# nmdp-bioinformatics/py-graph-imputation

Hardware: NVIDIA B200
Metric: subjects_per_sec (higher is better)
Workload: dtype f64

## Files before the change

py-graph-imputation_b200/csrc/grimb200.cu:

```cuda
#include <cuda_runtime.h>
#include <cub/cub.cuh>

#include <chrono>
#include <cstdio>
#include <cstring>
#include <mutex>
#include <string>
#include <vector>

#include "grimb_plan.h"

using namespace grimb;

static thread_local std::string g_err;
static int fail(int code, const std::string& msg) {
  g_err = msg;
  return code;
}
#define CK(call)                                                                          \
  do {                                                                                    \
    cudaError_t e_ = (call);                                                              \
    if (e_ != cudaSuccess)                                                                \
      return fail(GRIMB_E_CUDA, std::string(#call) + ": " + cudaGetErrorString(e_));      \
  } while (0)
// ... 1655 lines not shown
    }
    const bool drain_now = qn >= PQ_DRAIN;
    if (drain_now) drain_issue(q, X, qh, qn, lane, d);
    uint32_t p1[2];
#pragma unroll
    for (int u = 0; u < 2; ++u) {
      p1[u] = GRIMB_NONE;
      bool more = pr[u] && fidx_step(w[u], key[u], sec[u], true, p1[u]);
      while (more) {
        sec[u] = (sec[u] + 1) & X.sec_mask;
        fidx_sector(X.keys + 4ull * sec[u], w[u]);
        more = fidx_step(w[u], key[u], sec[u], false, p1[u]);
      }
    }
    const bool last = stride >= S - s0;
#pragma unroll
    for (int u = 0; u < 2; ++u) {
      nf[u] = 0x8000u;
      if (!last && S - s0 - stride > (uint32_t)(2 * u + half)) {
        nk[u] = __ldg(reinterpret_cast<const uint4*>(B.packed_keys) + s0 + stride + 2 * u + half);
        nf[u] = B.packed_flags[s0 + stride + 2 * u + half];
      }
    }
    if (drain_now) {
      const uint32_t n = drain_finish(q, d, X, qh, mid, worklist, worklist_n, extra, extra_n, extra_cap, lane);
      qh += n;
      qn -= n;
      __syncwarp();
    }
    uint32_t base = qh + qn;
#pragma unroll
    for (int u = 0; u < 2; ++u) {
      const uint32_t s = s0 + 2 * u + half;
      const uint32_t fl = cf[u];
      const bool inb = S - s0 > (uint32_t)(2 * u + half);
      const bool shape = inb && !(fl & 0x8000u) && nchain_ok;
      const bool same = (fl & 31u) == 0u;
      const bool hit = p1[u] != GRIMB_NONE;
      const uint32_t enq = __ballot_sync(FULL, hit && !same);
      const uint32_t hh = (enq >> (half << 4)) & 0xFFFFu;
      if (hit && !same) {
        const uint32_t e = (base + __popc(enq & lt)) & (PQ_CAP - 1u);
        q.key[e] = key2[u];
        q.p1[e] = p1[u];
        q.s[e] = s;
        q.ph[e] = (uint8_t)i;
      }
      base += __popc(enq);
      if (i == 0 && inb) {
        if (!shape) {
          if (fl & 0x8000u)
            O.r.compact[s] = make_compact(GRIMB_ST_SKIPPED, GRIMB_KIND_GENERAL, 0, 0xFFFFFFFFu, 0.0);
          else
            worklist[atomicAdd(worklist_n, 1u)] = s;
          mid.head[s] = FastHead{0u, 0u, make_uint2(0u, 0u)};
        } else if (same) {
          mid.head[s] = FastHead{1u | (hit ? (1u << 2) | (1u << 16) : 0u) | (1u << 7), 0u, make_uint2(p1[u], p1[u])};
        } else if (hh == 0u) {
          mid.head[s] = FastHead{1u, 0u, make_uint2(0u, 0u)};
        }
      }
    }
    qn = base - qh;
    __syncwarp();
    while (qn >= PQ_HIGH) {
      drain_issue(q, X, qh, qn, lane, d);
      const uint32_t n = drain_finish(q, d, X, qh, mid, worklist, worklist_n, extra, extra_n, extra_cap, lane);
      qh += n;
      qn -= n;
      __syncwarp();
    }
    if (last) break;
    s0 += stride;
  }
  while (qn > 0) {
    drain_issue(q, X, qh, qn, lane, d);
    const uint32_t n = drain_finish(q, d, X, qh, mid, worklist, worklist_n, extra, extra_n, extra_cap, lane);
    qh += n;
    qn -= n;
    __syncwarp();
  }
}

struct LongCand {
  FastPair pr;
  double p;
  bool valid;
};

__device__ __forceinline__ void long_cand(LongCand& c, const FastExtra* ex, const double* __restrict__ fslot, uint32_t q,
                                          uint32_t ncand, double m, bool same) {
  c.valid = q < ncand;
  double2 v = make_double2(0.0, 0.0);
  if (c.valid) {
    const uint2 pp = ex->p[q];
    v.x = __ldg(fslot + pp.x);
    v.y = __ldg(fslot + pp.y);
  }
  c.pr.f = v.x;
  c.pr.f2 = v.y;
  c.pr.same = same;
  c.pr.mpos = c.valid && m > 0;
  c.pr.y = m * c.pr.f2;
  const double t = fmin(c.pr.f2, same ? c.pr.y * 0.5 : c.pr.y);
  const double b = c.pr.f * t;
  const bool tiny = !(b > 1.0e-280);
  c.pr.lo = tiny ? -1.0 : b * (1.0 - 0x1p-50);
  c.pr.hi = tiny ? __longlong_as_double(0x7ff0000000000000LL) : b * (1.0 + 0x1p-50);
  c.p = v.x * v.y * m;
  if (!same) c.p = c.p * 2;
}

__device__ __forceinline__ double shfl_double(double v, int src) {
  const long long b = __double_as_longlong(v);
  const int lo = __shfl_sync(0xFFFFFFFFu, (int)(b & 0xFFFFFFFFll), src), hi = __shfl_sync(0xFFFFFFFFu, (int)(b >> 32), src);
  return __longlong_as_double(((long long)hi << 32) | (unsigned int)lo);
}

struct ScoreLong {
  double total, e_fin;
  uint32_t n_acc, evals;
};

__device__ __noinline__ void score_long_eval(const FastExtra* ex, const double* fslot, uint32_t ncand, double m, bool same,
                                             const double* chain, int nchain, ScoreLong& o) {
  const int lane = threadIdx.x & 31;
  LongCand c;
  long_cand(c, ex, fslot, (uint32_t)lane, ncand, m, same);
  uint32_t rq = 99;
  if (c.pr.mpos) {
    int r = 0;
    while (r < nchain && chain[r] >= c.pr.hi) ++r;
    while (r < nchain && !c.pr.accept(chain[r])) ++r;
    if (r < nchain) rq = (uint32_t)r;
  }
  const uint32_t rs = __reduce_min_sync(0xFFFFFFFFu, rq);
  o.total = 0.0;
  o.e_fin = 0.0;
  o.n_acc = 0;
  if (rs == 99) {
    o.evals = ncand * (uint32_t)nchain;
    return;
  }
  o.evals = ncand * (rs + 1);
  bool acc = rq <= rs;
  if (chain[rs] > 0) {
    double mx = acc ? c.p : 0.0;
#pragma unroll
    for (int d = 16; d > 0; d >>= 1) {
      const double y = shfl_double(mx, lane ^ d);
      mx = y > mx ? y : mx;
    }
    o.e_fin = mx / 100000;
    acc = c.pr.accept(o.e_fin);
    o.evals += ncand;
  }
  uint32_t am = __ballot_sync(0xFFFFFFFFu, acc);
  o.n_acc = (uint32_t)__popc(am);
  bool first = true;
  while (am) {
    const int j = __ffs(am) - 1;
    am &= am - 1;
    const double pj = shfl_double(c.p, j);
    o.total = first ? pj : o.total + pj;
    first = false;
  }
}

__device__ __noinline__ void score_long_rows(const FastExtra* ex, const double* fslot, uint32_t ncand, double m, bool same,
                                             double e_fin, uint32_t cmask, uint32_t np, uint64_t* words) {
  const int lane = threadIdx.x & 31;
  LongCand c;
  long_cand(c, ex, fslot, (uint32_t)lane, ncand, m, same);
  const bool acc = c.pr.accept(e_fin);
  uint32_t am = __ballot_sync(0xFFFFFFFFu, acc);
  uint32_t rank = 0;
  while (am) {
    const int j = __ffs(am) - 1;
    am &= am - 1;
    const double pj = shfl_double(c.p, j);
    if (pj > c.p || (pj == c.p && j < lane)) ++rank;
  }
  uint32_t lo = 0, hi = 0;
  if (acc && rank < np) {
    const uint32_t id = __fns(cmask, 0, lane + 1) & 15u;
    if (rank < 8) lo = id << (4 * rank);
    else hi = id << (4 * (rank - 8));
    words[2 + rank] = (uint64_t)__double_as_longlong(c.p);
  }
  lo = __reduce_or_sync(0xFFFFFFFFu, lo);
  hi = __reduce_or_sync(0xFFFFFFFFu, hi);
  if (lane == 0) {
    words[0] = (uint64_t)np;
    words[1] = (uint64_t)lo | ((uint64_t)hi << 32);
  }
}

#ifndef FASTSCORE_MIN_BLOCKS
#define FASTSCORE_MIN_BLOCKS 8
#endif
__global__ void __launch_bounds__(128, FASTSCORE_MIN_BLOCKS)
k_fast_score(TablesView T, const FastIndex X, const GrimbConfig* __restrict__ cfg, GrimbBatch B, OutArrays O,
             const FastMid mid, const FastExtra* __restrict__ extra, uint32_t* worklist, unsigned int* worklist_n,
             uint32_t s_begin) {
  __shared__ double s_chain[FAST_MAX_ROUNDS];
  __shared__ int s_nchain;
  const int lane = threadIdx.x & 31;
  GrimbResults& R = O.r;
  const bool want_u = cfg->output_umug != 0, want_p = cfg->output_pmug != 0, planb = cfg->planb != 0;
  const uint32_t lim_r = (uint32_t)cfg->n_results;
  if (threadIdx.x == 0) {
    double e = cfg->epsilon;
    int n = 0;
    while (e > 0 && n < FAST_MAX_ROUNDS) {
      e /= 10;
      if (e < 1.0e-9) e = 0.0;
      s_chain[n++] = e;
    }
    s_nchain = (e > 0) ? -1 : n;
  }
  __syncthreads();
  const int nchain = s_nchain;
  const uint64_t S = (uint64_t)B.n_subjects;
  const uint64_t nthreads = (uint64_t)gridDim.x * blockDim.x;
  unsigned long long evals_sum = 0;
  for (uint64_t s0 = (uint64_t)s_begin + ((uint64_t)blockIdx.x * blockDim.x + threadIdx.x) - lane; s0 < S; s0 += nthreads) {
    const uint64_t s = s0 + lane;
    bool ready = false;
    double m = 0.0;
    uint32_t fl = 0, xslot = 0;
    uint32_t cmask = 0;
    uint2 p0 = make_uint2(0u, 0u);
    if (s < S) {
      const uint4 h1 = *reinterpret_cast<const uint4*>(mid.head + s);
      const uint32_t pi = batch_prior(B, s);
      m = __ldg(B.priors + pi);
      fl = h1.x;
      xslot = h1.y;
      p0 = make_uint2(h1.z, h1.w);
      cmask = fl >> 16;
      ready = (fl & 3u) == 1u;
    }
    const uint32_t ncand_all = ready ? ((fl >> 2) & 31u) : 0u;
    const bool long_form = ncand_all > (uint32_t)FAST_CMAX;
    const uint32_t ncand = long_form ? 0u : ncand_all;
    const bool same = (fl >> 7) & 1u;
    const bool mpos = m > 0;
    ScoreLong sl;
    sl.total = sl.e_fin = 0.0;
    sl.n_acc = sl.evals = 0;
    for (uint32_t lm = __ballot_sync(0xFFFFFFFFu, long_form); lm; lm &= lm - 1) {
      const int o = __ffs(lm) - 1;
      ScoreLong r;
      score_long_eval(extra + __shfl_sync(0xFFFFFFFFu, xslot, o), X.fslot, __shfl_sync(0xFFFFFFFFu, ncand_all, o), shfl_double(m, o),
                      __shfl_sync(0xFFFFFFFFu, (int)same, o) != 0, s_chain, nchain, r);
      if (lane == o) sl = r;
    }
    double pf[FAST_CMAX], pf2[FAST_CMAX], prob[FAST_CMAX];
    uint32_t rq[FAST_CMAX];
    bool acc[FAST_CMAX];
    uint32_t r_star = 99;
    uint2 pp[FAST_CMAX];
    pp[0] = p0;
#pragma unroll
    for (int q = 1; q < FAST_CMAX; ++q) pp[q] = (uint32_t)q < ncand ? mid.more[s].p[q - 1] : make_uint2(0u, 0u);
#pragma unroll
    for (int q = 0; q < FAST_CMAX; ++q) {
      pf[q] = pf2[q] = 0.0;
      if ((uint32_t)q < ncand) {
        pf[q] = __ldg(X.fslot + pp[q].x);
        pf2[q] = __ldg(X.fslot + pp[q].y);
      }
    }
#pragma unroll
    for (int q = 0; q < FAST_CMAX; ++q) {
      prob[q] = 0.0;
      rq[q] = 99;
      acc[q] = false;
      if ((uint32_t)q < ncand) {
        const double2 v = make_double2(pf[q], pf2[q]);
        FastPair pr;
        pr.f = v.x;
        pr.f2 = v.y;
        pr.same = same;
        pr.mpos = mpos;
        pr.y = m * pr.f2;
        const double t = fmin(pr.f2, same ? pr.y * 0.5 : pr.y);
        const double b = pr.f * t;
        const bool tiny = !(b > 1.0e-280);
        pr.lo = tiny ? -1.0 : b * (1.0 - 0x1p-50);
        pr.hi = tiny ? __longlong_as_double(0x7ff0000000000000LL) : b * (1.0 + 0x1p-50);
        double p = v.x * v.y * m;
        if (!same) p = p * 2;
        prob[q] = p;
        if (mpos) {
          int r = 0;
          while (r < nchain && s_chain[r] >= pr.hi) ++r;
          while (r < nchain && !pr.accept(s_chain[r])) ++r;
          if (r < nchain) rq[q] = (uint32_t)r;
        }
        r_star = rq[q] < r_star ? rq[q] : r_star;
      }
    }
    uint32_t evals = 0, n_acc = 0;
    if (r_star == 99) {
      evals = ncand * (uint32_t)nchain;
    } else {
      evals = ncand * (r_star + 1);
      if (s_chain[r_star] > 0) {
        double mx = 0.0;
#pragma unroll
        for (int q = 0; q < FAST_CMAX; ++q)
          if (rq[q] <= r_star && prob[q] > mx) mx = prob[q];
        const double eps = mx / 100000;
#pragma unroll
        for (int q = 0; q < FAST_CMAX; ++q)
          if ((uint32_t)q < ncand) {
            FastPair pr;
            pr.f = pf[q];
            pr.f2 = pf2[q];
            pr.same = same;
            pr.mpos = mpos;
            pr.y = m * pr.f2;
            const double t = fmin(pr.f2, same ? pr.y * 0.5 : pr.y);
            const double b = pr.f * t;
            const bool tiny = !(b > 1.0e-280);
            pr.lo = tiny ? -1.0 : b * (1.0 - 0x1p-50);
            pr.hi = tiny ? __longlong_as_double(0x7ff0000000000000LL) : b * (1.0 + 0x1p-50);
            acc[q] = pr.accept(eps);
          }
        evals += ncand;
      } else {
#pragma unroll
        for (int q = 0; q < FAST_CMAX; ++q) acc[q] = rq[q] <= r_star;
      }
    }
    double total = 0.0;
    bool first = true;
#pragma unroll
    for (int q = 0; q < FAST_CMAX; ++q)
      if (acc[q]) {
        total = first ? prob[q] : total + prob[q];
        first = false;
        ++n_acc;
      }
    if (long_form) {
      total = sl.total;
      n_acc = sl.n_acc;
      evals = sl.evals;
    }
    if (want_u && want_p) evals *= 2;
    bool done = ready;
    if (ready && n_acc == 0 && planb) {
      worklist[atomicAdd(worklist_n, 1u)] = (uint32_t)s;
      done = false;
    }
    if (done) evals_sum += evals;
    const uint32_t np = (done && n_acc != 0 && want_p) ? (n_acc < lim_r ? n_acc : lim_r) : 0u;
    const uint32_t nw = long_form ? (np ? np + 2u : 0u) : ((np != 0u && n_acc >= 2u) ? np : 0u);
    uint32_t sc = nw;
#pragma unroll
    for (int d = 1; d < 32; d <<= 1) {
      const uint32_t a = __shfl_up_sync(0xFFFFFFFFu, sc, d);
      if (lane >= d) sc += a;
    }
    const uint32_t wtot = __shfl_sync(0xFFFFFFFFu, sc, 31);
    unsigned long long wb = 0;
    if (wtot) {
      if (lane == 31) wb = atomicAdd(O.word_counter, (unsigned long long)wtot);
      wb = __shfl_sync(0xFFFFFFFFu, wb, 31);
    }
    const uint64_t my = wb + (sc - nw);
    const bool fits = (int64_t)(wb + wtot) <= R.word_capacity;
    for (uint32_t lm = __ballot_sync(0xFFFFFFFFu, long_form && done && np && fits); lm; lm &= lm - 1) {
      const int o = __ffs(lm) - 1;
      const uint32_t ph = __shfl_sync(0xFFFFFFFFu, cmask, o);
      const uint64_t at = (uint64_t)__shfl_sync(0xFFFFFFFFu, (uint32_t)my, o) |
                          ((uint64_t)__shfl_sync(0xFFFFFFFFu, (uint32_t)(my >> 32), o) << 32);
      score_long_rows(extra + __shfl_sync(0xFFFFFFFFu, xslot, o), X.fslot, __shfl_sync(0xFFFFFFFFu, ncand_all, o), shfl_double(m, o),
                      __shfl_sync(0xFFFFFFFFu, (int)same, o) != 0, shfl_double(sl.e_fin, o), ph, __shfl_sync(0xFFFFFFFFu, np, o),
                      R.words + at);
    }
    if (!done) continue;
    uint32_t phases = 0;
    uint32_t mm = cmask;
#pragma unroll
    for (int q = 0; q < FAST_CMAX; ++q) {
      const uint32_t pid = (uint32_t)(__ffs(mm) - 1) & 15u;
      mm &= mm - 1;
      if (acc[q]) {
        uint32_t rank = 0;
#pragma unroll
        for (int j = 0; j < FAST_CMAX; ++j)
          if (acc[j] && (prob[j] > prob[q] || (prob[j] == prob[q] && j < q))) ++rank;
        if (rank < np) {
          phases |= pid << (4 * rank);
          if (nw && fits) R.words[my + rank] = (uint64_t)__double_as_longlong(prob[q]);
        }
      }
    }
    const GrimbCompact c = make_compact(GRIMB_ST_OK, GRIMB_KIND_SIMPLE | (n_acc ? GRIMB_KIND_HAS_RESULTS : 0u) |
                                        (nw ? GRIMB_KIND_WORDS : 0u) | ((long_form ? (np ? 15u : 0u) : np) << 4), phases,
                                        (uint32_t)my, total);
    *reinterpret_cast<uint4*>(R.compact + s) = *reinterpret_cast<const uint4*>(&c);
  }
#pragma unroll
  for (int d = 16; d > 0; d >>= 1) evals_sum += __shfl_xor_sync(0xFFFFFFFFu, evals_sum, d);
  if (lane == 0 && evals_sum) atomicAdd(O.evals_counter, evals_sum);
}

#endif

constexpr int TY_WARPS = 8;
constexpr int TY_VP = 4;
#ifndef TY_MIN_BLOCKS
#define TY_MIN_BLOCKS 4
#endif
constexpr int TY_MAX_ROUNDS = 40;

struct __align__(16) TyLists {
  uint16_t ph[TY_VP];
  uint16_t ph_pad[4];
  double f1s[TY_VP][32];
  double f2s[TY_VP][32];
  double pm2[TY_VP][32];
  double xs[32];
  uint8_t p1s[TY_VP][32];
  uint8_t p2s[TY_VP][32];
  uint8_t n1[TY_VP], n2[TY_VP];
};

static inline size_t ty_bytes_per_warp(int P) {
  const size_t G = (size_t)P * (P + 1) / 2;
  return (sizeof(TyLists) + G * 12 + 15) & ~(size_t)15;
}

__global__ void __launch_bounds__(TY_WARPS * 32, TY_MIN_BLOCKS)
k_impute_typed(TablesView T, const GrimbConfig* __restrict__ cfg, GrimbBatch B, OutArrays O, uint32_t* worklist,
               unsigned int* worklist_n, uint32_t per_warp, uint32_t s_begin) {
  extern __shared__ __align__(16) unsigned char ty_smem[];
  __shared__ double s_chain[TY_MAX_ROUNDS];
  __shared__ int s_nchain;
  const uint32_t FULLM = 0xFFFFFFFFu;
  const int lane = threadIdx.x & 31, warp = threadIdx.x >> 5;
  const int L = T.L, P = T.P;
  const int G = P * (P + 1) / 2;
  TyLists& W = *reinterpret_cast<TyLists*>(ty_smem + (size_t)warp * per_warp);
  double* gsum = reinterpret_cast<double*>(ty_smem + (size_t)warp * per_warp + sizeof(TyLists));
  uint16_t* gslot = reinterpret_cast<uint16_t*>(gsum + G);
  uint16_t* gpair = gslot + G;
  GrimbResults& R = O.r;
  const bool want_u = cfg->output_umug != 0, want_p = cfg->output_pmug != 0;
  const uint32_t lim_r = (uint32_t)cfg->n_results, lim_p = (uint32_t)cfg->n_pop_results;
  const int K = cfg->max_haps_in_phase;
  if (threadIdx.x == 0) {
    double e = cfg->epsilon;
    int n = 0;
    while (e > 0 && n < TY_MAX_ROUNDS) {
      e /= 10;
      if (e < 1.0e-9) e = 0.0;
      s_chain[n++] = e;
    }
    s_nchain = (e > 0) ? -1 : n;
  }
  __syncthreads();
  const int nchain = s_nchain;
  const uint32_t full = (1u << L) - 1u;
  const uint32_t nphase = 1u << (L - 1);
  const uint64_t S = (uint64_t)B.n_subjects;
  unsigned long long evals_sum = 0;
  unsigned long long n_probes = 0, n_hits = 0, n_vecs = 0;
  for (uint64_t s = (uint64_t)s_begin + (uint64_t)blockIdx.x * TY_WARPS + warp; s < S; s += (uint64_t)gridDim.x * TY_WARPS) {
    const uint32_t typed = batch_typed(B, s, full);
    if (typed == 0) {
      if (lane == 0) R.compact[s] = make_compact(GRIMB_ST_SKIPPED, GRIMB_KIND_GENERAL, 0, 0xFFFFFFFFu, 0.0);
      continue;
    }
    const bool is_packed = B.packed_keys != nullptr;
    const uint32_t al_off = is_packed ? 0u : B.allele_off[s];
    const bool shape = typed == full && nchain >= 0 && (is_packed || B.allele_off[s + 1] - al_off == 2u * (uint32_t)L);
    uint32_t pairs[GRIMB_MAX_LOCI];
    uint32_t het = 0;
    if (shape) {
// ... 326 lines not shown
  out_idx[i] = s;
}

__global__ void k_snapshot(const unsigned long long* __restrict__ cnt, unsigned long long* out, int n) {
  if ((int)threadIdx.x < n) out[threadIdx.x] = cnt[threadIdx.x];
  __threadfence_system();
}

enum {
  CNT_WORK = 0,
  CNT_WORKLIST = 1,
  CNT_BUCKETS = 2,
  CNT_OVERFLOW = 4,
  CNT_SLOT_TICKET = 5,
  CNT_WORK2 = 6,
  CNT_CHUNK_END = 8,
  CNT_HAP = 8,
  CNT_POP = 9,
  CNT_WORDS = 10,
  CNT_GENERAL = 11,
  CNT_EVALS = 12,
  CNT_PROBES = 13,
  CNT_N = 16
};

struct GrimbEngine {
  const GrimbTables* tables;
  int device;
  int threads;
  int threads_fixed = 0;
  int64_t wide_cta_below = 2048;
  int split_heavy = 0;
  int n_ctas;
  uint64_t arena_per_cta;
  char* arena = nullptr;
  double* ones = nullptr;
  GrimbConfig* d_cfg = nullptr;
  unsigned long long* d_counters = nullptr;
  cudaStream_t stream = nullptr;
  cudaStream_t s_in = nullptr, s_out = nullptr;
  cudaEvent_t ev_in[GRIMB_MAX_CHUNKS], ev_k[GRIMB_MAX_CHUNKS];
  unsigned long long* h_cnt = nullptr;
  unsigned long long* h_cnt_dev = nullptr;
  int64_t host_chunk = 262144;
  GrimbConfig cfg_host;
  GrimbConfig cfg_dev;
  int cfg_sent = 0;
  unsigned long long* h_tail = nullptr;
  cudaStream_t pending_stream = nullptr;
  int pending = 0;
  cudaEvent_t ev_done = nullptr;
  int tail_queued = 0;
  int tail_expected = 0;
  GrimbBatch pend_batch;
  GrimbResults pend_res;
  int64_t launches = 0;
  DevBuf in[6], outb[5], in_mask;
  DevBuf worklist;
  DevBuf buckets;
  DevBuf gather;
  void* h_gather = nullptr;
  size_t h_gather_cap = 0;
  DevBuf pre_top, pre_meta;
  uint32_t pre_max = 0;
  int pre_K = 0;
  int sm_count = 0;
  int fast_path = 1;
  int fast_split = 1;
  int fast_probe = 2;
  int last_probe = -1;
  int timing = 1;
  int timing_host = 0;
  DevBuf mid;
  DevBuf overflow;
  cudaEvent_t ev_score[2] = {nullptr, nullptr};
  int ev_score_valid = 0;
  cudaEvent_t ev_slots[2] = {nullptr, nullptr};
  int ev_slots_valid = 0;
  cudaEvent_t ev[6] = {nullptr, nullptr, nullptr, nullptr, nullptr, nullptr};
  int ev_valid[3] = {0, 0, 0};
  double last_worklist = -1;
  int typed_ctas = 0;
  uint32_t typed_per_warp = 0;
  DevBuf geno_keys, geno_flags, geno_mask, geno_off, geno_alleles, geno_small, scan_tmp;
  unsigned long long* h_small = nullptr;
  cudaEvent_t ev_geno[4] = {nullptr, nullptr, nullptr, nullptr};
  int ev_geno_valid = 0;
  cudaEvent_t ev_rows[4] = {nullptr, nullptr, nullptr, nullptr};
  int ev_rows_valid = 0;
  DevBuf gl_in_off, gl_stage, gl_mask, gl_counts, gl_off, gl_alleles;
  cudaEvent_t ev_gl[4] = {nullptr, nullptr, nullptr, nullptr};
  int ev_gl_valid = 0;
};

extern "C" int grimb_engine_free(GrimbEngine* e);

static void set_l2_fetch_granularity() {
  const char* v = getenv("GRIMB_L2_FETCH");
  if (!v) return;
  const long x = atol(v);
  if (x != 32 && x != 64 && x != 128) return;
  if (cudaDeviceSetLimit(cudaLimitMaxL2FetchGranularity, (size_t)x) != cudaSuccess) cudaGetLastError();
}

extern "C" int grimb_engine_create(const GrimbTables* t, int64_t workspace_bytes_per_cta, GrimbEngine** out) {
  if (!t || !out || workspace_bytes_per_cta < (1 << 16)) return fail(GRIMB_E_ARG, "bad engine arguments");
  CK(cudaSetDevice(t->device));
  set_l2_fetch_granularity();
  GrimbEngine* e = new GrimbEngine();
  for (int i = 0; i < GRIMB_MAX_CHUNKS; ++i) e->ev_in[i] = e->ev_k[i] = nullptr;
  e->tables = t;
  e->device = t->device;
  e->threads = 128;
#define CKE(call)                                                                          \
  do {                                                                                     \
    cudaError_t e_ = (call);                                                               \
    if (e_ != cudaSuccess) {                                                               \
      grimb_engine_free(e);                                                                \
      return fail(GRIMB_E_CUDA, std::string(#call) + ": " + cudaGetErrorString(e_));       \
    }                                                                                      \
  } while (0)
  cudaDeviceProp prop;
  CKE(cudaGetDeviceProperties(&prop, t->device));
  int per_sm = 0;
  CKE(cudaOccupancyMaxActiveBlocksPerMultiprocessor(&per_sm, k_impute, e->threads, 0));
  if (per_sm < 1) per_sm = 1;
  size_t free_b = 0, total_b = 0;
  CKE(cudaMemGetInfo(&free_b, &total_b));
  int64_t n = (int64_t)prop.multiProcessorCount * per_sm;
  e->arena_per_cta = ((uint64_t)workspace_bytes_per_cta + 255ull) & ~255ull;
  while (n > prop.multiProcessorCount && (uint64_t)n * e->arena_per_cta > free_b / 2) n -= prop.multiProcessorCount;
  while (n > 1 && (uint64_t)n * e->arena_per_cta > free_b / 2) n /= 2;
  e->n_ctas = (int)n;
  cudaError_t ce = cudaMalloc((void**)&e->arena, (uint64_t)e->n_ctas * e->arena_per_cta);
  if (ce != cudaSuccess) {
    grimb_engine_free(e);
    return fail(GRIMB_E_NOMEM, std::string("engine arena: ") + cudaGetErrorString(ce));
  }
  const int P = t->h.P;
  std::vector<double> one((size_t)P * P, 1.0);
  CKE(cudaMalloc((void**)&e->ones, one.size() * 8));
  CKE(cudaMemcpy(e->ones, one.data(), one.size() * 8, cudaMemcpyHostToDevice));
  CKE(cudaMalloc((void**)&e->d_cfg, sizeof(GrimbConfig)));
  CKE(cudaMalloc((void**)&e->d_counters, CNT_N * sizeof(unsigned long long)));
  CKE(cudaStreamCreateWithFlags(&e->stream, cudaStreamNonBlocking));
  CKE(cudaStreamCreateWithFlags(&e->s_in, cudaStreamNonBlocking));
  CKE(cudaStreamCreateWithFlags(&e->s_out, cudaStreamNonBlocking));
  for (int i = 0; i < GRIMB_MAX_CHUNKS; ++i) {
    CKE(cudaEventCreateWithFlags(&e->ev_in[i], cudaEventDisableTiming));
    CKE(cudaEventCreateWithFlags(&e->ev_k[i], cudaEventDisableTiming));
  }
  CKE(cudaHostAlloc((void**)&e->h_cnt, (GRIMB_MAX_CHUNKS + 1) * CNT_N * sizeof(unsigned long long), cudaHostAllocMapped));
  CKE(cudaHostGetDevicePointer((void**)&e->h_cnt_dev, e->h_cnt, 0));
  CKE(cudaMallocHost((void**)&e->h_tail, CNT_N * sizeof(unsigned long long)));
  if (const char* hc = getenv("GRIMB_HOST_CHUNK")) {
    const long long v = atoll(hc);
    if (v >= 1024) e->host_chunk = v;
  }
  for (int i = 0; i < 6; ++i) CKE(cudaEventCreate(&e->ev[i]));
  e->sm_count = prop.multiProcessorCount;
  if (P <= 32) {
    e->typed_per_warp = (uint32_t)ty_bytes_per_warp(P);
    const size_t dyn = (size_t)e->typed_per_warp * TY_WARPS;
    CKE(cudaFuncSetAttribute(k_impute_typed, cudaFuncAttributeMaxDynamicSharedMemorySize,
                             (int)(ty_bytes_per_warp(32) * TY_WARPS)));
    int tb = 0;
    CKE(cudaOccupancyMaxActiveBlocksPerMultiprocessor(&tb, k_impute_typed, TY_WARPS * 32, dyn));
    e->typed_ctas = (tb < 1 ? 1 : tb) * prop.multiProcessorCount;
  }
  const char* fp = getenv("GRIMB_FAST");
  if (fp && fp[0] == '0') e->fast_path = 0;
  const char* fsp = getenv("GRIMB_FAST_SPLIT");
  if (fsp && fsp[0] == '0') e->fast_split = 0;
  const char* fpr = getenv("GRIMB_FAST_PROBE");
  if (fpr && fpr[0] == '1') e->fast_probe = 1;
  const char* kev = getenv("GRIMB_KERNEL_EVENTS");
  if (kev && kev[0] == '0') e->timing = 0;
  const char* hev = getenv("GRIMB_HOST_EVENTS");
  if (hev && hev[0] == '1') e->timing_host = 1;
  for (int i = 0; i < 2; ++i) CKE(cudaEventCreate(&e->ev_score[i]));
  for (int i = 0; i < 2; ++i) CKE(cudaEventCreate(&e->ev_slots[i]));
  CKE(cudaEventCreateWithFlags(&e->ev_done, cudaEventDisableTiming));
  for (int i = 0; i < 4; ++i) CKE(cudaEventCreate(&e->ev_geno[i]));
  for (int i = 0; i < 4; ++i) CKE(cudaEventCreate(&e->ev_rows[i]));
  for (int i = 0; i < 4; ++i) CKE(cudaEventCreate(&e->ev_gl[i]));
  CKE(cudaMallocHost((void**)&e->h_small, 8 * sizeof(unsigned long long)));
  e->pre_max = 4096;
  if (const char* gs = getenv("GRIMB_GROUP_SUBJECTS")) {
    const long long v = atoll(gs);
    if (v >= 0 && v <= (1 << 20)) e->pre_max = (uint32_t)v;
  }
  const char* th = getenv("GRIMB_THREADS");
  if (th) {
    int v = atoi(th);
    if (v >= 32 && v <= MAXT && v % 32 == 0) {
      e->threads = v;
      e->threads_fixed = 1;
    }
  }
  if (const char* wc = getenv("GRIMB_WIDE_CTA_BELOW")) e->wide_cta_below = atoll(wc);
  if (const char* sh = getenv("GRIMB_SPLIT_HEAVY")) {
    const int v = atoi(sh);
    if (v >= 0 && v < GRIMB_BUCKETS) e->split_heavy = v;
  }
#undef CKE
  *out = e;
  return GRIMB_OK;
}

extern "C" int grimb_engine_free(GrimbEngine* e) {
  if (!e) return GRIMB_OK;
  cudaSetDevice(e->device);
  if (e->stream) cudaStreamSynchronize(e->stream);
  cudaFree(e->arena);
  cudaFree(e->ones);
  cudaFree(e->d_cfg);
  cudaFree(e->d_counters);
  if (e->stream) cudaStreamDestroy(e->stream);
  if (e->s_in) cudaStreamDestroy(e->s_in);
  if (e->s_out) cudaStreamDestroy(e->s_out);
  for (int i = 0; i < GRIMB_MAX_CHUNKS; ++i) {
    if (e->ev_in[i]) cudaEventDestroy(e->ev_in[i]);
    if (e->ev_k[i]) cudaEventDestroy(e->ev_k[i]);
  }
  for (int i = 0; i < 6; ++i)
    if (e->ev[i]) cudaEventDestroy(e->ev[i]);
  for (int i = 0; i < 2; ++i)
    if (e->ev_score[i]) cudaEventDestroy(e->ev_score[i]);
  for (int i = 0; i < 2; ++i)
    if (e->ev_slots[i]) cudaEventDestroy(e->ev_slots[i]);
  if (e->ev_done) cudaEventDestroy(e->ev_done);
  for (int i = 0; i < 4; ++i) {
    if (e->ev_geno[i]) cudaEventDestroy(e->ev_geno[i]);
    if (e->ev_rows[i]) cudaEventDestroy(e->ev_rows[i]);
    if (e->ev_gl[i]) cudaEventDestroy(e->ev_gl[i]);
  }
  if (e->h_small) cudaFreeHost(e->h_small);
  if (e->h_gather) cudaFreeHost(e->h_gather);
  if (e->h_cnt) cudaFreeHost(e->h_cnt);
  if (e->h_tail) cudaFreeHost(e->h_tail);
  cudaGetLastError();
  delete e;
  return GRIMB_OK;
}

extern "C" int64_t grimb_engine_launches(const GrimbEngine* e) { return e ? e->launches : 0; }

extern "C" double grimb_engine_kernel_ms(const GrimbEngine* e, int which) {
  if (e && which == 3) return e->last_worklist;
  if (e && which == 6) return (double)e->last_probe;
  if (e && which >= 7 && which <= 9) {
    const cudaEvent_t* ev = which == 7 ? e->ev_geno : which == 8 ? e->ev_rows : e->ev_gl;
// ... 54 lines not shown
  CK(cudaStreamSynchronize(e->stream));
  e->cfg_host = *cfg;
  e->cfg_dev = *cfg;
  if (cfg->plan_a_only) e->cfg_dev.planb = 0;
  CK(cudaMemcpyAsync(e->d_cfg, &e->cfg_dev, sizeof(GrimbConfig), cudaMemcpyHostToDevice, st));
  CK(cudaStreamSynchronize(st));
  e->cfg_sent = 1;
  return GRIMB_OK;
}

static OutArrays out_arrays(GrimbEngine* e, const GrimbResults& r) {
  OutArrays O;
  O.r = r;
  O.hap_counter = e->d_counters + CNT_HAP;
  O.pop_counter = e->d_counters + CNT_POP;
  O.word_counter = e->d_counters + CNT_WORDS;
  O.general_counter = e->d_counters + CNT_GENERAL;
  O.evals_counter = e->d_counters + CNT_EVALS;
  O.probe_counters = e->d_counters + CNT_PROBES;
  return O;
}

static bool warp_kernels_apply(const GrimbEngine* e, const GrimbConfig* cfg, const GrimbBatch* batch) {
  if (!(e->fast_path && (!batch->phase_mask || batch->packed_keys) && !cfg->hap_pop_pair && !cfg->encounter_order)) return false;
  const TablesView& tv = e->tables->view;
#if GRIMB_KW == 1
  if (tv.L <= 5 && tv.P == 1) return true;
#endif
  return e->typed_ctas > 0;
}

static int launch_warp(GrimbEngine* e, const GrimbConfig* cfg, const GrimbBatch* batch, const OutArrays& O, cudaStream_t st,
                       bool tm, int64_t s_begin, int64_t s_end) {
  const int64_t n = s_end - s_begin;
  if (n <= 0 || !warp_kernels_apply(e, cfg, batch)) return GRIMB_OK;
  const TablesView& tv = e->tables->view;
  GrimbBatch rb = *batch;
  rb.n_subjects = s_end;
  CK(e->worklist.reserve((size_t)batch->n_subjects * 4 + 16));
  unsigned int* cnt = (unsigned int*)(e->d_counters + CNT_WORKLIST);
#if GRIMB_KW == 1
  if (tv.L <= 5 && tv.P == 1) {
    const uint64_t groups = ((uint64_t)n + FAST_WARPS * 2 - 1) / (FAST_WARPS * 2);
    if (e->fast_split) {
      const FastIndex& fidx = e->tables->fidx;
      if (!fidx.keys) return fail(GRIMB_E_ARG, "table has no fast-path index");
      CK(e->mid.reserve((size_t)batch->n_subjects * (sizeof(FastHead) + sizeof(FastMore)) + 256));
      FastMid midv;
      midv.head = (FastHead*)e->mid.p;
      midv.more = (FastMore*)((char*)e->mid.p + (((size_t)batch->n_subjects * sizeof(FastHead) + 127) & ~(size_t)127));
      double eps = cfg->epsilon;
      int nr = 0;
      while (eps > 0 && nr < FAST_MAX_ROUNDS) {
        eps /= 10;
        if (eps < 1.0e-9) eps = 0.0;
        ++nr;
      }
      uint64_t fgp = (uint64_t)e->sm_count * FASTPROBE_MIN_BLOCKS;
      if (fgp > groups) fgp = groups;
      const uint32_t extra_cap = (uint32_t)(batch->n_subjects / 16 + 1024);
      CK(e->overflow.reserve((size_t)extra_cap * sizeof(FastExtra) + 64));
      unsigned int* ovf_n = (unsigned int*)(e->d_counters + CNT_OVERFLOW);
      if (tm) CK(cudaEventRecord(e->ev[0], st));
      if (batch->packed_keys && e->fast_probe == 2) {
        uint64_t g2 = (uint64_t)e->sm_count * FASTPROBE2_MIN_BLOCKS;
        const uint64_t quads = ((uint64_t)n + FAST_WARPS * 4 - 1) / (FAST_WARPS * 4);
        if (g2 > quads) g2 = quads;
        k_fast_probe2<<<(unsigned)g2, FAST_WARPS * 32, 0, st>>>(tv, fidx, rb, O, midv, (uint32_t*)e->worklist.p, cnt,
                                                             (FastExtra*)e->overflow.p, ovf_n, extra_cap, eps > 0 ? 0 : 1,
                                                             (uint32_t)s_begin);
        e->last_probe = 2;
      } else if (batch->packed_keys) {
        k_fast_probe<true><<<(unsigned)fgp, FAST_WARPS * 32, 0, st>>>(tv, fidx, rb, O, midv, (uint32_t*)e->worklist.p, cnt,
                                                                    (FastExtra*)e->overflow.p, ovf_n, extra_cap, eps > 0 ? 0 : 1, (uint32_t)s_begin);
        e->last_probe = 1;
      } else {
        k_fast_probe<false><<<(unsigned)fgp, FAST_WARPS * 32, 0, st>>>(tv, fidx, rb, O, midv, (uint32_t*)e->worklist.p, cnt,
                                                                     (FastExtra*)e->overflow.p, ovf_n, extra_cap, eps > 0 ? 0 : 1, (uint32_t)s_begin);
        e->last_probe = 0;
      }
      CK(cudaGetLastError());
      if (tm) CK(cudaEventRecord(e->ev[1], st));
      uint64_t sg = ((uint64_t)n + 127) / 128;
      if (sg > (uint64_t)e->sm_count * 16) sg = (uint64_t)e->sm_count * 16;
      if (tm) CK(cudaEventRecord(e->ev_score[0], st));
      k_fast_score<<<(unsigned)sg, 128, 0, st>>>(tv, fidx, e->d_cfg, rb, O, midv, (const FastExtra*)e->overflow.p,
                                                (uint32_t*)e->worklist.p, cnt, (uint32_t)s_begin);
      CK(cudaGetLastError());
      if (tm) CK(cudaEventRecord(e->ev_score[1], st));
      e->ev_score_valid = tm;
      e->ev_valid[0] = tm;
      e->launches += 2;
    } else {
      uint64_t fg = (uint64_t)e->sm_count * FAST_MIN_BLOCKS;
      if (fg > groups) fg = groups;
      if (tm) CK(cudaEventRecord(e->ev[0], st));
      k_impute_fast<false><<<(unsigned)fg, FAST_WARPS * 32, 0, st>>>(tv, e->d_cfg, rb, O, (uint32_t*)e->worklist.p, cnt, nullptr,
                                                                    nullptr, (uint32_t)s_begin);
      CK(cudaGetLastError());
      if (tm) CK(cudaEventRecord(e->ev[1], st));
      e->ev_valid[0] = tm;
      e->launches += 1;
    }
    return GRIMB_OK;
  }
#endif
  uint64_t tg = ((uint64_t)n + TY_WARPS - 1) / TY_WARPS;
  if (tg > (uint64_t)e->typed_ctas) tg = (uint64_t)e->typed_ctas;
  if (tm) CK(cudaEventRecord(e->ev[4], st));
  k_impute_typed<<<(unsigned)tg, TY_WARPS * 32, (size_t)e->typed_per_warp * TY_WARPS, st>>>(
      tv, e->d_cfg, rb, O, (uint32_t*)e->worklist.p, cnt, e->typed_per_warp, (uint32_t)s_begin);
  CK(cudaGetLastError());
  if (tm) CK(cudaEventRecord(e->ev[5], st));
  e->ev_valid[2] = tm;
  e->launches += 1;
  return GRIMB_OK;
}

static int launch_tail(GrimbEngine* e, const GrimbConfig* cfg, const GrimbBatch* batch, const OutArrays& O, cudaStream_t st,
                       bool tm, int64_t n_tail = -1) {
  if (batch->n_subjects <= 0) return GRIMB_OK;
  const TablesView& tv = e->tables->view;
  const bool warp = warp_kernels_apply(e, cfg, batch);
  const uint32_t* wl = warp ? (const uint32_t*)e->worklist.p : nullptr;
  unsigned int* cnt = (unsigned int*)(e->d_counters + CNT_WORKLIST);
  const unsigned int* wl_n = warp ? cnt : nullptr;
  const uint64_t stride = (uint64_t)batch->n_subjects;
  CK(e->buckets.reserve((size_t)stride * 4 * GRIMB_BUCKETS + 16));
  unsigned int* bucket_n = (unsigned int*)(e->d_counters + CNT_BUCKETS);
  {
    uint64_t cg = (stride + 255) / 256;
    if (cg > (uint64_t)e->sm_count * 4) cg = (uint64_t)e->sm_count * 4;
    if (wl) cg = cg < 64 ? cg : 64;
    k_classify<<<(unsigned)cg, 256, 0, st>>>(*batch, tv.L, wl, wl_n, (uint32_t*)e->buckets.p, bucket_n, stride);
    CK(cudaGetLastError());
    e->launches += 1;
  }
  int grid = e->n_ctas;
  if ((int64_t)grid > batch->n_subjects) grid = (int)batch->n_subjects;
  int threads = e->threads;
  if (!e->threads_fixed && n_tail >= 0 && n_tail <= e->wide_cta_below && e->n_ctas >= 4) {
    threads = n_tail <= e->wide_cta_below / 8 ? 512 : 256;
    const int div = threads / 128;
    if (grid > e->n_ctas / div) grid = e->n_ctas / div;
  }
  PreView pv;
  memset(&pv, 0, sizeof(pv));
  if (e->pre_max > 0 && (!batch->phase_mask || batch->packed_keys)) {
    const uint32_t spp = 1u << tv.L;
    const uint32_t K = (uint32_t)cfg->max_haps_in_phase;
    uint64_t fit = e->pre_max;
    const uint64_t budget = 1ull << 31;
    const uint64_t per_subject = (uint64_t)spp * K * sizeof(TopItem);
    if (fit * per_subject > budget) fit = budget / per_subject;
    if ((int64_t)fit > batch->n_subjects) fit = (uint64_t)batch->n_subjects;
    if (fit > 0) {
      CK(e->pre_top.reserve(fit * per_subject + 16));
      CK(e->pre_meta.reserve(fit * spp * 12 + 16));
      pv.top = (TopItem*)e->pre_top.p;
      pv.n = (uint32_t*)e->pre_meta.p;
      pv.ne = pv.n + fit * spp;
      pv.ready = pv.ne + fit * spp;
      pv.max_subjects = (uint32_t)fit;
      pv.slots_per_subject = spp;
      pv.K = K;
      if (tm) CK(cudaEventRecord(e->ev_slots[0], st));
      k_impute<<<grid, threads, 0, st>>>(tv, e->d_cfg, *batch, O, e->arena, e->arena_per_cta, e->ones,
// ... 931 lines not shown
```

Measured before the change: 4.843 billion.

## Score multi-candidate subjects warp-cooperatively and size score grid by occupancy

Each thread now scores single-candidate subjects inline. Every subject with two or more candidates, short or long form, goes through a warp-cooperative loop in which each lane handles one candidate. This replaces the per-thread unrolled FAST_CMAX arrays and the rank loops, which should cut register pressure and divergence. The change also switches subject indices to 32-bit, skips the word-offset scan when no lane needs words, lowers the launch-bounds min blocks from 8 to 6, and sets the score grid from measured occupancy. The trade-off is more warp-serialised work when many subjects in a warp have multiple candidates.

```diff
diff --git a/py-graph-imputation_b200/csrc/grimb200.cu b/py-graph-imputation_b200/csrc/grimb200.cu
--- a/py-graph-imputation_b200/csrc/grimb200.cu
+++ b/py-graph-imputation_b200/csrc/grimb200.cu
@@ -1761,33 +1761,51 @@
   }
 }
 
-struct LongCand {
+__device__ __forceinline__ FastPair fast_pair(double f, double f2, double m, bool same) {
+  FastPair pr;
+  pr.f = f;
+  pr.f2 = f2;
+  pr.same = same;
+  pr.mpos = m > 0;
+  pr.y = m * f2;
+  const double t = fmin(f2, same ? pr.y * 0.5 : pr.y);
+  const double b = f * t;
+  const bool tiny = !(b > 1.0e-280);
+  pr.lo = tiny ? -1.0 : b * (1.0 - 0x1p-50);
+  pr.hi = tiny ? __longlong_as_double(0x7ff0000000000000LL) : b * (1.0 + 0x1p-50);
+  return pr;
+}
+
+__device__ __forceinline__ double fast_prob(double f, double f2, double m, bool same) {
+  double p = f * f2 * m;
+  if (!same) p = p * 2;
+  return p;
+}
+
+__device__ __forceinline__ uint32_t first_round(const FastPair& pr, const double* chain, int nchain) {
+  if (!pr.mpos) return 99;
+  int r = 0;
+  while (r < nchain && chain[r] >= pr.hi) ++r;
+  while (r < nchain && !pr.accept(chain[r])) ++r;
+  return r < nchain ? (uint32_t)r : 99u;
+}
+
+struct MultiCand {
   FastPair pr;
   double p;
-  bool valid;
 };
 
-__device__ __forceinline__ void long_cand(LongCand& c, const FastExtra* ex, const double* __restrict__ fslot, uint32_t q,
-                                          uint32_t ncand, double m, bool same) {
-  c.valid = q < ncand;
-  double2 v = make_double2(0.0, 0.0);
-  if (c.valid) {
-    const uint2 pp = ex->p[q];
-    v.x = __ldg(fslot + pp.x);
-    v.y = __ldg(fslot + pp.y);
-  }
-  c.pr.f = v.x;
-  c.pr.f2 = v.y;
-  c.pr.same = same;
-  c.pr.mpos = c.valid && m > 0;
-  c.pr.y = m * c.pr.f2;
-  const double t = fmin(c.pr.f2, same ? c.pr.y * 0.5 : c.pr.y);
-  const double b = c.pr.f * t;
-  const bool tiny = !(b > 1.0e-280);
-  c.pr.lo = tiny ? -1.0 : b * (1.0 - 0x1p-50);
-  c.pr.hi = tiny ? __longlong_as_double(0x7ff0000000000000LL) : b * (1.0 + 0x1p-50);
-  c.p = v.x * v.y * m;
-  if (!same) c.p = c.p * 2;
+__device__ __forceinline__ void multi_cand(MultiCand& c, const uint2* first, const uint2* rest, const double* __restrict__ fslot,
+                                           uint32_t q, uint32_t ncand, double m, bool same) {
+  double f = 0.0, f2 = 0.0;
+  if (q < ncand) {
+    const uint2 pp = q == 0 ? *first : rest[q - 1];
+    f = __ldg(fslot + pp.x);
+    f2 = __ldg(fslot + pp.y);
+  }
+  c.pr = fast_pair(f, f2, m, same);
+  c.pr.mpos = q < ncand && m > 0;
+  c.p = fast_prob(f, f2, m, same);
 }
 
 __device__ __forceinline__ double shfl_double(double v, int src) {
@@ -1796,23 +1814,17 @@
   return __longlong_as_double(((long long)hi << 32) | (unsigned int)lo);
 }
 
-struct ScoreLong {
+struct ScoreMulti {
   double total, e_fin;
   uint32_t n_acc, evals;
 };
 
-__device__ __noinline__ void score_long_eval(const FastExtra* ex, const double* fslot, uint32_t ncand, double m, bool same,
-                                             const double* chain, int nchain, ScoreLong& o) {
+__device__ __forceinline__ void score_multi_eval(const uint2* first, const uint2* rest, const double* fslot, uint32_t ncand,
+                                              double m, bool same, const double* chain, int nchain, ScoreMulti& o) {
   const int lane = threadIdx.x & 31;
-  LongCand c;
-  long_cand(c, ex, fslot, (uint32_t)lane, ncand, m, same);
-  uint32_t rq = 99;
-  if (c.pr.mpos) {
-    int r = 0;
-    while (r < nchain && chain[r] >= c.pr.hi) ++r;
-    while (r < nchain && !c.pr.accept(chain[r])) ++r;
-    if (r < nchain) rq = (uint32_t)r;
-  }
+  MultiCand c;
+  multi_cand(c, first, rest, fslot, (uint32_t)lane, ncand, m, same);
+  const uint32_t rq = first_round(c.pr, chain, nchain);
   const uint32_t rs = __reduce_min_sync(0xFFFFFFFFu, rq);
   o.total = 0.0;
   o.e_fin = 0.0;
@@ -1836,21 +1848,22 @@
   }
   uint32_t am = __ballot_sync(0xFFFFFFFFu, acc);
   o.n_acc = (uint32_t)__popc(am);
-  bool first = true;
+  bool first_acc = true;
   while (am) {
     const int j = __ffs(am) - 1;
     am &= am - 1;
     const double pj = shfl_double(c.p, j);
-    o.total = first ? pj : o.total + pj;
-    first = false;
-  }
-}
-
-__device__ __noinline__ void score_long_rows(const FastExtra* ex, const double* fslot, uint32_t ncand, double m, bool same,
-                                             double e_fin, uint32_t cmask, uint32_t np, uint64_t* words) {
+    o.total = first_acc ? pj : o.total + pj;
+    first_acc = false;
+  }
+}
+
+__device__ __forceinline__ uint64_t score_multi_rows(const uint2* first, const uint2* rest, const double* fslot, uint32_t ncand,
+                                                  double m, bool same, double e_fin, uint32_t cmask, uint32_t np,
+                                                  uint64_t* words, bool long_form) {
   const int lane = threadIdx.x & 31;
-  LongCand c;
-  long_cand(c, ex, fslot, (uint32_t)lane, ncand, m, same);
+  MultiCand c;
+  multi_cand(c, first, rest, fslot, (uint32_t)lane, ncand, m, same);
   const bool acc = c.pr.accept(e_fin);
   uint32_t am = __ballot_sync(0xFFFFFFFFu, acc);
   uint32_t rank = 0;
@@ -1865,18 +1878,20 @@
     const uint32_t id = __fns(cmask, 0, lane + 1) & 15u;
     if (rank < 8) lo = id << (4 * rank);
     else hi = id << (4 * (rank - 8));
-    words[2 + rank] = (uint64_t)__double_as_longlong(c.p);
+    if (words) words[(long_form ? 2 : 0) + rank] = (uint64_t)__double_as_longlong(c.p);
   }
   lo = __reduce_or_sync(0xFFFFFFFFu, lo);
   hi = __reduce_or_sync(0xFFFFFFFFu, hi);
-  if (lane == 0) {
+  const uint64_t ids = (uint64_t)lo | ((uint64_t)hi << 32);
+  if (long_form && lane == 0) {
     words[0] = (uint64_t)np;
-    words[1] = (uint64_t)lo | ((uint64_t)hi << 32);
-  }
+    words[1] = ids;
+  }
+  return ids;
 }
 
 #ifndef FASTSCORE_MIN_BLOCKS
-#define FASTSCORE_MIN_BLOCKS 8
+#define FASTSCORE_MIN_BLOCKS 6
 #endif
 __global__ void __launch_bounds__(128, FASTSCORE_MIN_BLOCKS)
 k_fast_score(TablesView T, const FastIndex X, const GrimbConfig* __restrict__ cfg, GrimbBatch B, OutArrays O,
@@ -1884,6 +1899,7 @@
              uint32_t s_begin) {
   __shared__ double s_chain[FAST_MAX_ROUNDS];
   __shared__ int s_nchain;
+  const uint32_t FULL = 0xFFFFFFFFu;
   const int lane = threadIdx.x & 31;
   GrimbResults& R = O.r;
   const bool want_u = cfg->output_umug != 0, want_p = cfg->output_pmug != 0, planb = cfg->planb != 0;
@@ -1900,184 +1916,114 @@
   }
   __syncthreads();
   const int nchain = s_nchain;
-  const uint64_t S = (uint64_t)B.n_subjects;
-  const uint64_t nthreads = (uint64_t)gridDim.x * blockDim.x;
+  const uint32_t S = (uint32_t)B.n_subjects;
+  const uint32_t nthreads = gridDim.x * blockDim.x;
   unsigned long long evals_sum = 0;
-  for (uint64_t s0 = (uint64_t)s_begin + ((uint64_t)blockIdx.x * blockDim.x + threadIdx.x) - lane; s0 < S; s0 += nthreads) {
-    const uint64_t s = s0 + lane;
-    bool ready = false;
+  for (uint32_t s0 = s_begin + (blockIdx.x * blockDim.x + threadIdx.x) - lane; s0 < S; s0 += nthreads) {
+    const uint32_t s = s0 + lane;
     double m = 0.0;
     uint32_t fl = 0, xslot = 0;
-    uint32_t cmask = 0;
     uint2 p0 = make_uint2(0u, 0u);
     if (s < S) {
       const uint4 h1 = *reinterpret_cast<const uint4*>(mid.head + s);
-      const uint32_t pi = batch_prior(B, s);
-      m = __ldg(B.priors + pi);
+      m = __ldg(B.priors + batch_prior(B, s));
       fl = h1.x;
       xslot = h1.y;
       p0 = make_uint2(h1.z, h1.w);
-      cmask = fl >> 16;
-      ready = (fl & 3u) == 1u;
-    }
-    const uint32_t ncand_all = ready ? ((fl >> 2) & 31u) : 0u;
-    const bool long_form = ncand_all > (uint32_t)FAST_CMAX;
-    const uint32_t ncand = long_form ? 0u : ncand_all;
+    }
+    const bool ready = (fl & 3u) == 1u;
+    const uint32_t ncand = ready ? ((fl >> 2) & 31u) : 0u;
+    const uint32_t cmask = fl >> 16;
     const bool same = (fl >> 7) & 1u;
-    const bool mpos = m > 0;
-    ScoreLong sl;
-    sl.total = sl.e_fin = 0.0;
-    sl.n_acc = sl.evals = 0;
-    for (uint32_t lm = __ballot_sync(0xFFFFFFFFu, long_form); lm; lm &= lm - 1) {
+    const bool multi = ncand >= 2u;
+    double f = 0.0, f2 = 0.0;
+    if (ncand == 1u) {
+      f = __ldg(X.fslot + p0.x);
+      f2 = __ldg(X.fslot + p0.y);
+    }
+    uint32_t evals = 0, n_acc = 0;
+    double total = 0.0;
+    if (ncand == 1u) {
+      const FastPair pr = fast_pair(f, f2, m, same);
+      const double p = fast_prob(f, f2, m, same);
+      const uint32_t r = first_round(pr, s_chain, nchain);
+      if (r == 99) {
+        evals = (uint32_t)nchain;
+      } else {
+        evals = r + 1;
+        bool acc = true;
+        if (s_chain[r] > 0) {
+          const double mx = p > 0.0 ? p : 0.0;
+          acc = pr.accept(mx / 100000);
+          evals += 1;
+        }
+        if (acc) {
+          total = p;
+          n_acc = 1;
+        }
+      }
+    }
+    ScoreMulti sm;
+    sm.total = sm.e_fin = 0.0;
+    sm.n_acc = sm.evals = 0;
+    for (uint32_t lm = __ballot_sync(FULL, multi); lm; lm &= lm - 1) {
       const int o = __ffs(lm) - 1;
-      ScoreLong r;
-      score_long_eval(extra + __shfl_sync(0xFFFFFFFFu, xslot, o), X.fslot, __shfl_sync(0xFFFFFFFFu, ncand_all, o), shfl_double(m, o),
-                      __shfl_sync(0xFFFFFFFFu, (int)same, o) != 0, s_chain, nchain, r);
-      if (lane == o) sl = r;
-    }
-    double pf[FAST_CMAX], pf2[FAST_CMAX], prob[FAST_CMAX];
-    uint32_t rq[FAST_CMAX];
-    bool acc[FAST_CMAX];
-    uint32_t r_star = 99;
-    uint2 pp[FAST_CMAX];
-    pp[0] = p0;
-#pragma unroll
-    for (int q = 1; q < FAST_CMAX; ++q) pp[q] = (uint32_t)q < ncand ? mid.more[s].p[q - 1] : make_uint2(0u, 0u);
-#pragma unroll
-    for (int q = 0; q < FAST_CMAX; ++q) {
-      pf[q] = pf2[q] = 0.0;
-      if ((uint32_t)q < ncand) {
-        pf[q] = __ldg(X.fslot + pp[q].x);
-        pf2[q] = __ldg(X.fslot + pp[q].y);
-      }
-    }
-#pragma unroll
-    for (int q = 0; q < FAST_CMAX; ++q) {
-      prob[q] = 0.0;
-      rq[q] = 99;
-      acc[q] = false;
-      if ((uint32_t)q < ncand) {
-        const double2 v = make_double2(pf[q], pf2[q]);
-        FastPair pr;
-        pr.f = v.x;
-        pr.f2 = v.y;
-        pr.same = same;
-        pr.mpos = mpos;
-        pr.y = m * pr.f2;
-        const double t = fmin(pr.f2, same ? pr.y * 0.5 : pr.y);
-        const double b = pr.f * t;
-        const bool tiny = !(b > 1.0e-280);
-        pr.lo = tiny ? -1.0 : b * (1.0 - 0x1p-50);
-        pr.hi = tiny ? __longlong_as_double(0x7ff0000000000000LL) : b * (1.0 + 0x1p-50);
-        double p = v.x * v.y * m;
-        if (!same) p = p * 2;
-        prob[q] = p;
-        if (mpos) {
-          int r = 0;
-          while (r < nchain && s_chain[r] >= pr.hi) ++r;
-          while (r < nchain && !pr.accept(s_chain[r])) ++r;
-          if (r < nchain) rq[q] = (uint32_t)r;
-        }
-        r_star = rq[q] < r_star ? rq[q] : r_star;
-      }
-    }
-    uint32_t evals = 0, n_acc = 0;
-    if (r_star == 99) {
-      evals = ncand * (uint32_t)nchain;
-    } else {
-      evals = ncand * (r_star + 1);
-      if (s_chain[r_star] > 0) {
-        double mx = 0.0;
-#pragma unroll
-        for (int q = 0; q < FAST_CMAX; ++q)
-          if (rq[q] <= r_star && prob[q] > mx) mx = prob[q];
-        const double eps = mx / 100000;
-#pragma unroll
-        for (int q = 0; q < FAST_CMAX; ++q)
-          if ((uint32_t)q < ncand) {
-            FastPair pr;
-            pr.f = pf[q];
-            pr.f2 = pf2[q];
-            pr.same = same;
-            pr.mpos = mpos;
-            pr.y = m * pr.f2;
-            const double t = fmin(pr.f2, same ? pr.y * 0.5 : pr.y);
-            const double b = pr.f * t;
-            const bool tiny = !(b > 1.0e-280);
-            pr.lo = tiny ? -1.0 : b * (1.0 - 0x1p-50);
-            pr.hi = tiny ? __longlong_as_double(0x7ff0000000000000LL) : b * (1.0 + 0x1p-50);
-            acc[q] = pr.accept(eps);
-          }
-        evals += ncand;
-      } else {
-#pragma unroll
-        for (int q = 0; q < FAST_CMAX; ++q) acc[q] = rq[q] <= r_star;
-      }
-    }
-    double total = 0.0;
-    bool first = true;
-#pragma unroll
-    for (int q = 0; q < FAST_CMAX; ++q)
-      if (acc[q]) {
-        total = first ? prob[q] : total + prob[q];
-        first = false;
-        ++n_acc;
-      }
-    if (long_form) {
-      total = sl.total;
-      n_acc = sl.n_acc;
-      evals = sl.evals;
+      const uint32_t nc = __shfl_sync(FULL, ncand, o);
+      const bool lf = nc > (uint32_t)FAST_CMAX;
+      const uint32_t x = __shfl_sync(FULL, xslot, o);
+      const uint2* first = lf ? extra[x].p : &mid.head[s0 + o].p0;
+      const uint2* rest = lf ? extra[x].p + 1 : mid.more[s0 + o].p;
+      ScoreMulti r;
+      score_multi_eval(first, rest, X.fslot, nc, shfl_double(m, o), __shfl_sync(FULL, (int)same, o) != 0, s_chain, nchain, r);
+      if (lane == o) sm = r;
+    }
+    if (multi) {
+      total = sm.total;
+      n_acc = sm.n_acc;
+      evals = sm.evals;
     }
     if (want_u && want_p) evals *= 2;
     bool done = ready;
     if (ready && n_acc == 0 && planb) {
-      worklist[atomicAdd(worklist_n, 1u)] = (uint32_t)s;
+      worklist[atomicAdd(worklist_n, 1u)] = s;
       done = false;
     }
     if (done) evals_sum += evals;
     const uint32_t np = (done && n_acc != 0 && want_p) ? (n_acc < lim_r ? n_acc : lim_r) : 0u;
+    const bool long_form = ncand > (uint32_t)FAST_CMAX;
     const uint32_t nw = long_form ? (np ? np + 2u : 0u) : ((np != 0u && n_acc >= 2u) ? np : 0u);
-    uint32_t sc = nw;
+    uint64_t my = 0;
+    bool fits = true;
+    if (__any_sync(FULL, nw != 0u)) {
+      uint32_t sc = nw;
 #pragma unroll
-    for (int d = 1; d < 32; d <<= 1) {
-      const uint32_t a = __shfl_up_sync(0xFFFFFFFFu, sc, d);
-      if (lane >= d) sc += a;
-    }
-    const uint32_t wtot = __shfl_sync(0xFFFFFFFFu, sc, 31);
-    unsigned long long wb = 0;
-    if (wtot) {
+      for (int d = 1; d < 32; d <<= 1) {
+        const uint32_t a = __shfl_up_sync(FULL, sc, d);
+        if (lane >= d) sc += a;
+      }
+      const uint32_t wtot = __shfl_sync(FULL, sc, 31);
+      unsigned long long wb = 0;
       if (lane == 31) wb = atomicAdd(O.word_counter, (unsigned long long)wtot);
-      wb = __shfl_sync(0xFFFFFFFFu, wb, 31);
-    }
-    const uint64_t my = wb + (sc - nw);
-    const bool fits = (int64_t)(wb + wtot) <= R.word_capacity;
-    for (uint32_t lm = __ballot_sync(0xFFFFFFFFu, long_form && done && np && fits); lm; lm &= lm - 1) {
+      wb = __shfl_sync(FULL, wb, 31);
+      my = wb + (sc - nw);
+      fits = (int64_t)(wb + wtot) <= R.word_capacity;
+    }
+    uint32_t phases = (ncand == 1u && np != 0u) ? ((uint32_t)(__ffs(cmask) - 1) & 15u) : 0u;
+    for (uint32_t lm = __ballot_sync(FULL, multi && np && (fits || !long_form)); lm; lm &= lm - 1) {
       const int o = __ffs(lm) - 1;
-      const uint32_t ph = __shfl_sync(0xFFFFFFFFu, cmask, o);
-      const uint64_t at = (uint64_t)__shfl_sync(0xFFFFFFFFu, (uint32_t)my, o) |
-                          ((uint64_t)__shfl_sync(0xFFFFFFFFu, (uint32_t)(my >> 32), o) << 32);
-      score_long_rows(extra + __shfl_sync(0xFFFFFFFFu, xslot, o), X.fslot, __shfl_sync(0xFFFFFFFFu, ncand_all, o), shfl_double(m, o),
-                      __shfl_sync(0xFFFFFFFFu, (int)same, o) != 0, shfl_double(sl.e_fin, o), ph, __shfl_sync(0xFFFFFFFFu, np, o),
-                      R.words + at);
+      const uint32_t nc = __shfl_sync(FULL, ncand, o);
+      const bool lf = nc > (uint32_t)FAST_CMAX;
+      const uint32_t x = __shfl_sync(FULL, xslot, o);
+      const uint2* first = lf ? extra[x].p : &mid.head[s0 + o].p0;
+      const uint2* rest = lf ? extra[x].p + 1 : mid.more[s0 + o].p;
+      const uint64_t at = (uint64_t)__shfl_sync(FULL, (uint32_t)my, o) | ((uint64_t)__shfl_sync(FULL, (uint32_t)(my >> 32), o) << 32);
+      const bool w = __shfl_sync(FULL, (int)(nw != 0u && fits), o) != 0;
+      const uint64_t ids = score_multi_rows(first, rest, X.fslot, nc, shfl_double(m, o), __shfl_sync(FULL, (int)same, o) != 0,
+                                            shfl_double(sm.e_fin, o), __shfl_sync(FULL, cmask, o), __shfl_sync(FULL, np, o),
+                                            w ? R.words + at : nullptr, lf);
+      if (lane == o && !lf) phases = (uint32_t)ids;
     }
     if (!done) continue;
-    uint32_t phases = 0;
-    uint32_t mm = cmask;
-#pragma unroll
-    for (int q = 0; q < FAST_CMAX; ++q) {
-      const uint32_t pid = (uint32_t)(__ffs(mm) - 1) & 15u;
-      mm &= mm - 1;
-      if (acc[q]) {
-        uint32_t rank = 0;
-#pragma unroll
-        for (int j = 0; j < FAST_CMAX; ++j)
-          if (acc[j] && (prob[j] > prob[q] || (prob[j] == prob[q] && j < q))) ++rank;
-        if (rank < np) {
-          phases |= pid << (4 * rank);
-          if (nw && fits) R.words[my + rank] = (uint64_t)__double_as_longlong(prob[q]);
-        }
-      }
-    }
     const GrimbCompact c = make_compact(GRIMB_ST_OK, GRIMB_KIND_SIMPLE | (n_acc ? GRIMB_KIND_HAS_RESULTS : 0u) |
                                         (nw ? GRIMB_KIND_WORDS : 0u) | ((long_form ? (np ? 15u : 0u) : np) << 4), phases,
                                         (uint32_t)my, total);
@@ -2570,6 +2516,7 @@
   double last_worklist = -1;
   int typed_ctas = 0;
   uint32_t typed_per_warp = 0;
+  int score_ctas = 0;
   DevBuf geno_keys, geno_flags, geno_mask, geno_off, geno_alleles, geno_small, scan_tmp;
   unsigned long long* h_small = nullptr;
   cudaEvent_t ev_geno[4] = {nullptr, nullptr, nullptr, nullptr};
@@ -2656,6 +2603,13 @@
     CKE(cudaOccupancyMaxActiveBlocksPerMultiprocessor(&tb, k_impute_typed, TY_WARPS * 32, dyn));
     e->typed_ctas = (tb < 1 ? 1 : tb) * prop.multiProcessorCount;
   }
+#if GRIMB_KW == 1
+  {
+    int sb = 0;
+    CKE(cudaOccupancyMaxActiveBlocksPerMultiprocessor(&sb, k_fast_score, 128, 0));
+    e->score_ctas = (sb < 1 ? 1 : sb) * prop.multiProcessorCount;
+  }
+#endif
   const char* fp = getenv("GRIMB_FAST");
   if (fp && fp[0] == '0') e->fast_path = 0;
   const char* fsp = getenv("GRIMB_FAST_SPLIT");
@@ -2876,7 +2830,7 @@
       CK(cudaGetLastError());
       if (tm) CK(cudaEventRecord(e->ev[1], st));
       uint64_t sg = ((uint64_t)n + 127) / 128;
-      if (sg > (uint64_t)e->sm_count * 16) sg = (uint64_t)e->sm_count * 16;
+      if (sg > (uint64_t)e->score_ctas) sg = (uint64_t)e->score_ctas;
       if (tm) CK(cudaEventRecord(e->ev_score[0], st));
       k_fast_score<<<(unsigned)sg, 128, 0, st>>>(tv, fidx, e->d_cfg, rb, O, midv, (const FastExtra*)e->overflow.p,
                                                 (uint32_t*)e->worklist.p, cnt, (uint32_t)s_begin);
```

After: 4.966 billion, median of 6. 1.03x the previous value.
